# VGLoic/kzg-poly-commit-exploration

Hardware: AMD Instinct MI355X
Metric: g1_msm_commitments_per_sec_degree_2^20 (higher is better)
Workload: dtype i32 digits (Fp: 13 signed radix-2^30 digits, Montgomery 2^390; Fr: 8 x u32, Montgomery 2^256)

## Files before the change

__graft_entry__.py:

```python
import os
import subprocess
import sys

ROOT = os.path.dirname(os.path.abspath(__file__))
sys.path.insert(0, ROOT)
sys.path.insert(0, os.path.join(ROOT, "oracle"))


def build():
    csrc = os.path.join(ROOT, "kzg_poly_commit_exploration_amd", "csrc")
    jobs = str(min(8, os.cpu_count() or 1))
    subprocess.run(["make", "-s", "-C", csrc, "-j", jobs], check=True)
    subprocess.run(["make", "-s", "-C", os.path.join(ROOT, "tests", "device")], check=True)
    subprocess.run(["make", "-s", "-C", os.path.join(ROOT, "tests", "device_columns")], check=True)
    subprocess.run(["make", "-s", "-C", os.path.join(ROOT, "oracle")], check=True)
    for example in ("commit_open", "open_points", "open_combined", "open_sets", "perm_quotient"):
        subprocess.run(["g++", "-std=c++17", "-I" + os.path.join(ROOT, "include"),
                        os.path.join(ROOT, "examples", example + ".cpp"),
                        "-L" + os.path.join(ROOT, "kzg_poly_commit_exploration_amd"), "-lkzg_mi355x",
                        "-Wl,-rpath,$ORIGIN/../kzg_poly_commit_exploration_amd",
                        "-o", os.path.join(ROOT, "examples", example)], check=True)
    import kzg_poly_commit_exploration_amd as K

    K.load_library()


def smoke():
    import numpy as np

    import bigint_twin as T
    import kzg_poly_commit_exploration_amd as K
    import oracle_ctypes as O

    d = 300
    eng = K.SetupArtifactsGenerator(T.BENCH_SECRET_BE).take(d + 1)
    try:
        c = O.bench_coefficients(d + 1)
        z = O.bench_input_point(d)
        y = O.poly_evaluate(c, z)
        srs = O.srs_g1(d + 1, T.BENCH_SECRET_BE)
        rc, want_c = O.commit_naive(c, srs)
        assert rc == 0
        rc, want_p = O.generate_proof(c, z, y, srs)
        assert rc == 0
        poly = K.Polynomial.from_limbs(c)
        got_c = poly.commit(eng)
        got_p = K.Evaluation(K.Scalar.from_limbs(z), K.Scalar.from_limbs(y)).generate_proof(poly, eng)
        assert got_c.compress() == O.p1_compress(want_c), "commitment differs from the oracle"
        assert got_p.compress() == O.p1_compress(want_p), "proof differs from the oracle"
        print("smoke ok: degree %d commit %s proof %s" % (d, got_c.compress().hex()[:16], got_p.compress().hex()[:16]))
    finally:
        eng.close()


if __name__ == "__main__":
    build()
    if len(sys.argv) > 1 and sys.argv[1] == "smoke":
        smoke()
```

kzg_poly_commit_exploration_amd/csrc/msm_sort.hip:

```cpp
#include <cstdlib>
#include <cstring>
#include <type_traits>

#include "engine.h"
#include "fr30.hip.h"
#include "msm_recode.h"

namespace kzg {

typedef uint32_t u32;
#ifndef KZG_DEV
#define KZG_DEV __device__ __forceinline__
#endif

static uint32_t ilog2(uint32_t v) {
    uint32_t b = 0;
    while ((1u << b) < v) b++;
    return b;
}

MsmConfig choose_msm_config(size_t n, size_t table_budget_bytes) {
    const char* force_mode = std::getenv("KZG_MSM_RECODE");
    const char* force_c = std::getenv("KZG_MSM_C");
    const uint32_t fc = force_c ? (uint32_t)std::strtoul(force_c, nullptr, 10) : 0u;
    const bool naf = force_mode && !std::strcmp(force_mode, "naf") && n * 255ull < 0x80000000ull &&
                     (double)n * 255.0 * (double)kAffineBytes <= (double)table_budget_bytes;
    uint32_t best_c = 8;
    const uint32_t best_mode = naf ? kRecodeNaf : kRecodeWindows;
    double best = 1e300;
    for (uint32_t c = 8; c <= (naf ? 21u : 20u); c++) {
        if (fc >= 8 && fc <= (naf ? 21u : 20u) && c != fc) continue;
        if (!naf && !fc && 254u - c * ((255 + c - 1) / c - 1) < 4u) continue;
        double cost = naf ? (double)n * (255.0 / (c + 1) + 0.5) + 8.0 * (double)(1u << (c - 2))
                          : (double)n * ((255 + c - 1) / c) + 20.0 * (double)(1u << (c - 1));
        if (cost < best) {
            best = cost;
            best_c = c;
        }
    }
    MsmConfig cfg;
    cfg.recode = best_mode;
    cfg.c = best_c;
    if (best_mode == kRecodeNaf) {
        cfg.W = 255;
        cfg.level_bits = 1;
        cfg.nb = 1u << (best_c - 2);
        cfg.max_digits = (255 + best_c - 1) / best_c + 1;
    } else {
        cfg.W = (255 + best_c - 1) / best_c;
        cfg.level_bits = best_c;
        cfg.nb = 1u << (best_c - 1);
        cfg.max_digits = cfg.W;
    }
    return cfg;
}

// ... 77 lines not shown
    uint32_t fine_bits = sort_fine_bits(cfg, false);
    uint32_t b = (uint32_t)kMaxCoarse / (cfg.nb >> fine_bits);
    return b < 1 ? 1 : b;
}

uint32_t sort_count_entries(uint32_t max_batch, MsmConfig cfg) {
    uint32_t bins = 0;
    for (uint32_t b = 1; b <= max_batch; b++) {
        const uint32_t nbt = cfg.nb * b;
        const uint32_t q = nbt >> sort_fine_bits(cfg, sort_packed_buckets(nbt, cfg));
        if (q > bins) bins = q;
    }
    return bins * (kMaxTiles + 1u);
}

struct BatchGeom {
    uint32_t n;
    uint32_t batch;
    uint64_t stride;
    uint32_t nb;
};

template <uint32_t C>
__global__ void __launch_bounds__(kRecodeBlock) k_sort_count(const uint32_t* __restrict__ d_scalars, int is_mont,
                                                           BatchGeom bg, MsmConfig cfg, uint32_t tile,
                                                           uint32_t fine_bits, uint32_t coarse_bins,
                                                           uint32_t* __restrict__ d_recoded ,
                                                           uint32_t* __restrict__ d_cnt, uint32_t* __restrict__ d_binfill ,
                                                           uint32_t* __restrict__ d_header) {
    __shared__ u32 s_hist[kMaxCoarse];
    if (blockIdx.x == 0 && threadIdx.x < kHeavyHeaderBytes / 4) d_header[threadIdx.x] = 0;
    for (uint32_t q = threadIdx.x; q < coarse_bins; q += kRecodeBlock) s_hist[q] = 0;
    __syncthreads();
    const uint64_t base = (uint64_t)blockIdx.x * tile;
    const uint64_t total = (uint64_t)bg.n * bg.batch;
    for (uint32_t off = threadIdx.x; off < tile; off += kRecodeBlock) {
        uint64_t g = base + off;
        if (g >= total) break;
        uint32_t p = (uint32_t)(g / bg.n);
        uint32_t i = (uint32_t)(g - (uint64_t)p * bg.n);
        u32 k[8];
        const bool flip = load_scalar(d_scalars, p * bg.stride + i, is_mont, k);
        store_recoded(d_recoded, g, k, flip);
        const u32 pb = p * bg.nb;
        for_each_digit<C>(k, cfg, [&](uint32_t, u32 bkt, bool) { atomicAdd(&s_hist[(pb + bkt) >> fine_bits], 1u); });
    }
    __syncthreads();
    for (uint32_t q = threadIdx.x; q < coarse_bins; q += kRecodeBlock) {
        const u32 c = s_hist[q];
        d_cnt[(size_t)blockIdx.x * coarse_bins + q] = c ? atomicAdd(&d_binfill[q], c) : 0u;
    }
}

template <int N>
__device__ __forceinline__ u32 block_exclusive_scan_n(u32 v, u32* lds, u32& total);
__device__ __forceinline__ u32 block_exclusive_scan_256(u32 v, u32* lds, u32& total);

constexpr uint32_t kFineMaxChunks = 4096;
constexpr uint32_t kFineLocal = 16;
constexpr uint32_t kWsBinStart = 0;
constexpr uint32_t kWsPrefix = kMaxCoarse + 8;
constexpr uint32_t kWsBinFill = 2 * kMaxCoarse + 32;
constexpr uint32_t kWsTable = 3 * kMaxCoarse + 64;
uint32_t sort_workspace_words() { return kWsTable + kFineMaxChunks * (uint32_t)kFineMax + 64; }
uint32_t sort_workspace_zero_words() { return kWsTable; }

template <int BLOCK>
KZG_DEV void spread_tile_cursors(uint32_t coarse_bins, const uint32_t* __restrict__ d_cnt, const uint32_t* __restrict__ d_binfill,
                                 uint32_t ch, uint32_t* __restrict__ d_binstart, uint32_t* __restrict__ d_prefix,
                                 uint32_t* __restrict__ d_total, u32* s_cur , u32* s_scan ) {
    const uint32_t t = threadIdx.x;
    constexpr uint32_t kStripes = kMaxCoarse / BLOCK;
    u32 below[kStripes], all[kStripes];
#pragma unroll
    for (uint32_t s = 0; s < kStripes; s++) {
        const uint32_t q = t + s * BLOCK;
        all[s] = q < coarse_bins ? d_binfill[q] : 0u;
        below[s] = q < coarse_bins ? d_cnt[(size_t)blockIdx.x * coarse_bins + q] : 0u;
    }
    u32 carry = 0, chunk_carry = 0;
#pragma unroll
    for (uint32_t s = 0; s < kStripes; s++) {
        if (s * BLOCK >= coarse_bins) break;
        const uint32_t q = t + s * BLOCK;
        u32 stripe_total;
        const u32 start = carry + block_exclusive_scan_n<BLOCK>(all[s], s_scan, stripe_total);
        __syncthreads();
        if (q < coarse_bins) s_cur[q] = start + below[s];
        if (blockIdx.x == 0) {
            const u32 nch = q < coarse_bins ? (all[s] + ch - 1) / ch : 0u;
            u32 chunk_total;
            const u32 cstart = chunk_carry + block_exclusive_scan_n<BLOCK>(nch, s_scan, chunk_total);
            __syncthreads();
            if (q < coarse_bins) {
                d_binstart[q] = start;
                d_prefix[q] = cstart;
            }
            chunk_carry += chunk_total;
        }
        carry += stripe_total;
    }
    if (blockIdx.x == 0 && t == 0) {
        d_binstart[coarse_bins] = carry;
        d_prefix[coarse_bins] = chunk_carry;
        *d_total = carry;
    }
    __syncthreads();
}

template <uint32_t C>
__global__ void __launch_bounds__(kRecodeBlock) k_sort_spread(const uint32_t* __restrict__ d_recoded,
                                                            BatchGeom bg, uint32_t table_stride, MsmConfig cfg,
                                                            uint32_t tile, uint32_t tiles, uint32_t fine_bits,
                                                            uint32_t coarse_bins, const uint32_t* __restrict__ d_cnt ,
                                                            const uint32_t* __restrict__ d_binfill ,
                                                            uint32_t ch, uint32_t* __restrict__ d_binstart,
                                                            uint32_t* __restrict__ d_prefix, uint32_t* __restrict__ d_total,
                                                            uint64_t* __restrict__ d_pairs, int packed) {
    __shared__ u32 s_cur[kMaxCoarse];
    __shared__ u32 s_scan[kRecodeBlock];
    spread_tile_cursors<kRecodeBlock>(coarse_bins, d_cnt, d_binfill, ch, d_binstart, d_prefix, d_total, s_cur, s_scan);
    const uint64_t base = (uint64_t)blockIdx.x * tile;
    const uint64_t total = (uint64_t)bg.n * bg.batch;
    const u32 fine_mask = (1u << fine_bits) - 1u;
    for (uint32_t off = threadIdx.x; off < tile; off += kRecodeBlock) {
        uint64_t g = base + off;
        if (g >= total) break;
        uint32_t p = (uint32_t)(g / bg.n);
        uint32_t i = (uint32_t)(g - (uint64_t)p * bg.n);
        u32 k[8];
        const bool flip = load_recoded(d_recoded, g, k);
        const u32 pb = p * bg.nb;
        for_each_digit<C>(k, cfg, [&](uint32_t j, u32 bkt, bool neg) {
            u32 b = pb + bkt;
            u32 pos = atomicAdd(&s_cur[b >> fine_bits], 1u);
            u32 ref = (j * table_stride + i) | ((neg != flip) ? 0x80000000u : 0u);
            if (packed) reinterpret_cast<u32*>(d_pairs)[pos] = ref | ((b & fine_mask) << kPackedIndexBits);
            else d_pairs[pos] = ((uint64_t)(b & fine_mask) << 32) | ref;
        });
    }
}

constexpr int kStageBlock = 512;
constexpr uint32_t kStageSlots = 7680;

template <int BLOCK>
KZG_DEV u32 block_exclusive_scan_fast(u32 v, u32* s_wave , u32& total) {
    const uint32_t t = threadIdx.x, lane = t & 63u, w = t >> 6;
    u32 incl = v;
#pragma unroll
    for (uint32_t off = 1; off < 64; off <<= 1) {
        const u32 up = __shfl_up(incl, off, 64);
        if (lane >= off) incl += up;
    }
    if (lane == 63) s_wave[w] = incl;
    __syncthreads();
    u32 base = 0, all = 0;
#pragma unroll
    for (uint32_t i = 0; i < BLOCK / 64; i++) {
        const u32 x = s_wave[i];
        if (i < w) base += x;
        all += x;
    }
    __syncthreads();
    total = all;
    return base + incl - v;
}

template <uint32_t C>
__global__ void __launch_bounds__(kStageBlock) k_sort_spread_staged(const uint32_t* __restrict__ d_recoded,
                                                                  BatchGeom bg, uint32_t table_stride, MsmConfig cfg,
                                                                  uint32_t tile, uint32_t fine_bits, uint32_t coarse_bins,
                                                                  const uint32_t* __restrict__ d_cnt, const uint32_t* __restrict__ d_binfill,
                                                                  uint32_t ch, uint32_t* __restrict__ d_binstart,
                                                                  uint32_t* __restrict__ d_prefix, uint32_t* __restrict__ d_total,
                                                                  uint32_t* __restrict__ d_pairs32) {
    __shared__ u32 s_cur[kMaxCoarse];
    __shared__ u32 s_cnt[kMaxCoarse];
    __shared__ u32 s_gd[kMaxCoarse];
    __shared__ u32 s_scan[kStageBlock];
    __shared__ u32 s_stage[kStageSlots];
    __shared__ uint16_t s_sbin[kStageSlots];
    spread_tile_cursors<kStageBlock>(coarse_bins, d_cnt, d_binfill, ch, d_binstart, d_prefix, d_total, s_cur, s_scan);
    const uint32_t t = threadIdx.x;
    const uint64_t base = (uint64_t)blockIdx.x * tile;
    const uint64_t total = (uint64_t)bg.n * bg.batch;
    const u32 fine_mask = (1u << fine_bits) - 1u;
    const uint32_t per_round = kStageSlots / cfg.max_digits < (uint32_t)kStageBlock ? kStageSlots / cfg.max_digits : (uint32_t)kStageBlock;
    constexpr uint32_t kBinsPerLane = kMaxCoarse / kStageBlock;
    for (uint32_t r0 = 0; r0 < tile; r0 += per_round) {
        for (uint32_t q = t; q < coarse_bins; q += kStageBlock) s_cnt[q] = 0;
        __syncthreads();
        const uint32_t off = r0 + t;
        const uint64_t g = base + off;
        const bool valid = t < per_round && off < tile && g < total;
        u32 k[8];
        bool flip = false;
        uint32_t i = 0;
        u32 pb = 0;
        if (valid) {
            const uint32_t p = (uint32_t)(g / bg.n);
            i = (uint32_t)(g - (uint64_t)p * bg.n);
            pb = p * bg.nb;
            flip = load_recoded(d_recoded, g, k);
            for_each_digit<C>(k, cfg, [&](uint32_t, u32 bkt, bool) { atomicAdd(&s_cnt[(pb + bkt) >> fine_bits], 1u); });
        }
        __syncthreads();
        u32 mine[kBinsPerLane], sum = 0;
#pragma unroll
        for (uint32_t e = 0; e < kBinsPerLane; e++) {
            const uint32_t q = t * kBinsPerLane + e;
            mine[e] = q < coarse_bins ? s_cnt[q] : 0u;
            sum += mine[e];
        }
        u32 round_total;
        u32 run = block_exclusive_scan_fast<kStageBlock>(sum, s_scan, round_total);
#pragma unroll
        for (uint32_t e = 0; e < kBinsPerLane; e++) {
            const uint32_t q = t * kBinsPerLane + e;
            if (q < coarse_bins) {
                const u32 cur = s_cur[q];
                s_gd[q] = cur - run;
                s_cur[q] = cur + mine[e];
                s_cnt[q] = run;
            }
            run += mine[e];
        }
        __syncthreads();
        if (valid) {
            for_each_digit<C>(k, cfg, [&](uint32_t j, u32 bkt, bool neg) {
                const u32 b = pb + bkt, bin = b >> fine_bits;
                const u32 slot = atomicAdd(&s_cnt[bin], 1u);
                s_stage[slot] = (j * table_stride + i) | ((neg != flip) ? 0x80000000u : 0u) | ((b & fine_mask) << kPackedIndexBits);
                s_sbin[slot] = (uint16_t)bin;
            });
        }
        __syncthreads();
        for (uint32_t e = t; e < round_total; e += kStageBlock) d_pairs32[s_gd[s_sbin[e]] + e] = s_stage[e];
    }
}


static uint32_t fine_chunk_len(uint64_t max_pairs) {
    static const uint64_t target = [] {
        const char* v = std::getenv("KZG_FINE_CHUNKS");
        uint64_t t = v ? std::strtoull(v, nullptr, 10) : 2048ull;
        return t < 1 ? 1ull : (t > 2048 ? 2048ull : t);
    }();
    uint64_t ch = (max_pairs + target - 1) / target;
    ch = (ch + 255) / 256 * 256;
    return (uint32_t)(ch < 4096 ? 4096 : ch);
}

struct FineChunk {
    uint32_t bin, beg, end, nch, j, base;
};
KZG_DEV bool locate_chunk(uint32_t k, const uint32_t* __restrict__ d_prefix, const uint32_t* __restrict__ d_binstart,
                          uint32_t coarse_bins, uint32_t ch, FineChunk& c) {
    if (k >= d_prefix[coarse_bins]) return false;
    uint32_t lo = 0, hi = coarse_bins;
    while (hi - lo > 1) {
        uint32_t mid = (lo + hi) >> 1;
        if (d_prefix[mid] <= k) lo = mid; else hi = mid;
    }
    c.bin = lo;
    c.base = d_prefix[lo];
    c.nch = d_prefix[lo + 1] - c.base;
    c.j = k - c.base;
    const uint32_t rs = d_binstart[lo], re = d_binstart[lo + 1];
    c.beg = rs + c.j * ch;
    c.end = (re - c.beg < ch) ? re : c.beg + ch;
    return true;
}

template <bool kPacked> struct SortPair;
template <> struct SortPair<false> {
    typedef uint64_t type;
    static KZG_DEV u32 key(uint64_t p) { return (u32)(p >> 32); }
    static KZG_DEV u32 ref(uint64_t p) { return (u32)p; }
};
template <> struct SortPair<true> {
    typedef uint32_t type;
    static KZG_DEV u32 key(uint32_t p) { return (p >> kPackedIndexBits) & ((1u << kPackedFineBits) - 1u); }
    static KZG_DEV u32 ref(uint32_t p) { return p & (0x80000000u | ((1u << kPackedIndexBits) - 1u)); }
};

template <bool kPacked>
__global__ void __launch_bounds__(kSortBlock) k_fine_count(const typename SortPair<kPacked>::type* __restrict__ d_pairs,
                                                           const uint32_t* __restrict__ d_binstart, uint32_t fine_bits,
                                                           uint32_t coarse_bins, uint32_t ch,
                                                           const uint32_t* __restrict__ d_prefix,
                                                           uint32_t* __restrict__ d_table, uint32_t* __restrict__ d_binfill) {
    __shared__ u32 s_hist[kFineMax];
    if (blockIdx.x == 0)
        for (uint32_t q = threadIdx.x; q < coarse_bins; q += kSortBlock) d_binfill[q] = 0;
    FineChunk c;
    if (!locate_chunk(blockIdx.x, d_prefix, d_binstart, coarse_bins, ch, c)) return;
    const uint32_t fine = 1u << fine_bits;
    if (threadIdx.x < fine) s_hist[threadIdx.x] = 0;
    __syncthreads();
    for (uint32_t e = c.beg + threadIdx.x; e < c.end; e += kSortBlock) atomicAdd(&s_hist[SortPair<kPacked>::key(d_pairs[e])], 1u);
    __syncthreads();
    if (threadIdx.x < fine) d_table[(size_t)c.base * fine + (size_t)threadIdx.x * c.nch + c.j] = s_hist[threadIdx.x];
}

__global__ void __launch_bounds__(kSortBlock) k_fine_binscan(const uint32_t* __restrict__ d_binstart, uint32_t fine_bits,
                                                             const uint32_t* __restrict__ d_prefix,
                                                             uint32_t* __restrict__ d_table, uint32_t* __restrict__ d_offs) {
    __shared__ u32 s_scan[kSortBlock];
    const uint32_t bin = blockIdx.x, t = threadIdx.x;
    const uint32_t fine = 1u << fine_bits;
    const uint32_t base = d_prefix[bin], nch = d_prefix[bin + 1] - base;
    const uint32_t rs = d_binstart[bin];
    if (nch == 0) {
        if (t < fine) d_offs[bin * fine + t] = rs;
        return;
    }
    if (nch <= kFineLocal) return;
    u32* h = d_table + (size_t)base * fine;
    const uint32_t len = fine * nch;
    const uint32_t per = (len + kSortBlock - 1) / kSortBlock;
    const uint32_t lo = t * per < len ? t * per : len, hi = lo + per < len ? lo + per : len;
    u32 sum = 0;
    for (uint32_t i = lo; i < hi; i++) sum += h[i];
    u32 total;
    u32 run = rs + block_exclusive_scan_256(sum, s_scan, total);
    for (uint32_t i = lo; i < hi; i++) {
        const u32 v = h[i];
        h[i] = run;
        run += v;
    }
}

constexpr uint32_t kFineStage = 4096;
template <bool kPacked>
__global__ void __launch_bounds__(kSortBlock) k_fine_scatter(const typename SortPair<kPacked>::type* __restrict__ d_pairs,
                                                             const uint32_t* __restrict__ d_binstart,
                                                             uint32_t fine_bits, uint32_t coarse_bins, uint32_t ch,
                                                             const uint32_t* __restrict__ d_prefix,
                                                             const uint32_t* __restrict__ d_table,
                                                             uint32_t* __restrict__ d_offs,
                                                             uint32_t* __restrict__ d_sorted) {
    __shared__ u32 s_cur[kFineMax];
    __shared__ u32 s_cnt[kFineMax];
    __shared__ u32 s_ref[kFineStage];
    __shared__ u32 s_dst[kFineStage];
    FineChunk c;
    if (!locate_chunk(blockIdx.x, d_prefix, d_binstart, coarse_bins, ch, c)) return;
    const uint32_t fine = 1u << fine_bits;
    const uint32_t t = threadIdx.x;
    {
        u32 mine = 0;
        if (c.nch <= kFineLocal) {
            u32 row = 0, front = 0;
            if (t < fine) {
                const u32* h = d_table + (size_t)c.base * fine + (size_t)t * c.nch;
                for (uint32_t i = 0; i < c.nch; i++) {
                    const u32 v = h[i];
                    row += v;
                    if (i < c.j) front += v;
                }
            }
            u32 total;
            const u32 key_start = d_binstart[c.bin] + block_exclusive_scan_256(row, s_ref, total);
            __syncthreads();
            mine = key_start + front;
            if (c.j == 0 && t < fine) d_offs[c.bin * fine + t] = key_start;
        } else if (t < fine) {
            mine = d_table[(size_t)c.base * fine + (size_t)t * c.nch + c.j];
            if (c.j == 0) d_offs[c.bin * fine + t] = mine;
        }
        if (t < fine) s_cur[t] = mine;
    }
    for (uint32_t r0 = c.beg; r0 < c.end; r0 += kFineStage) {
        const uint32_t r1 = (c.end - r0 < kFineStage) ? c.end : r0 + kFineStage;
        if (t < kFineMax) s_cnt[t] = 0;
        __syncthreads();
        typename SortPair<kPacked>::type pr[kFineStage / kSortBlock];
#pragma unroll
        for (uint32_t q = 0; q < kFineStage / kSortBlock; q++) {
            const uint32_t e = r0 + q * kSortBlock + t;
            pr[q] = e < r1 ? d_pairs[e] : (typename SortPair<kPacked>::type)0;
            if (e < r1) atomicAdd(&s_cnt[SortPair<kPacked>::key(pr[q])], 1u);
        }
        __syncthreads();
        u32 mine = t < kFineMax ? s_cnt[t] : 0u;
        u32 incl = mine;
        __syncthreads();
        if (t < kFineMax) s_ref[t] = incl;
        __syncthreads();
        for (uint32_t off = 1; off < kFineMax; off <<= 1) {
            u32 add = (t < kFineMax && t >= off) ? s_ref[t - off] : 0u;
            __syncthreads();
            if (t < kFineMax) {
                incl += add;
                s_ref[t] = incl;
            }
            __syncthreads();
        }
        const u32 excl = incl - mine;
        u32 gbase = 0;
        if (t < kFineMax) {
            gbase = s_cur[t];
            s_cur[t] = gbase + mine;
            s_cnt[t] = excl;
        }
        __syncthreads();
        if (t < kFineMax) s_dst[t] = gbase - excl;
        __syncthreads();
        u32 keep_dst[kFineStage / kSortBlock];
        u32 keep_pos[kFineStage / kSortBlock];
#pragma unroll
        for (uint32_t q = 0; q < kFineStage / kSortBlock; q++) {
            const uint32_t e = r0 + q * kSortBlock + t;
            if (e < r1) {
                const u32 key = SortPair<kPacked>::key(pr[q]);
                const u32 pos = atomicAdd(&s_cnt[key], 1u);
                keep_pos[q] = pos;
                keep_dst[q] = s_dst[key] + pos;
            }
        }
        __syncthreads();
#pragma unroll
        for (uint32_t q = 0; q < kFineStage / kSortBlock; q++) {
            const uint32_t e = r0 + q * kSortBlock + t;
            if (e < r1) {
                s_ref[keep_pos[q]] = SortPair<kPacked>::ref(pr[q]);
                s_dst[keep_pos[q]] = keep_dst[q];
            }
        }
        __syncthreads();
        const uint32_t cnt = r1 - r0;
        for (uint32_t i = t; i < cnt; i += kSortBlock) d_sorted[s_dst[i]] = s_ref[i];
        __syncthreads();
    }
}

template <int N>
__device__ __forceinline__ u32 block_exclusive_scan_n(u32 v, u32* lds, u32& total) {
    int t = threadIdx.x;
    lds[t] = v;
    __syncthreads();
    for (int off = 1; off < N; off <<= 1) {
        u32 add = t >= off ? lds[t - off] : 0u;
        __syncthreads();
        lds[t] += add;
        __syncthreads();
    }
    total = lds[N - 1];
    return lds[t] - v;
}
__device__ __forceinline__ u32 block_exclusive_scan_256(u32 v, u32* lds, u32& total) { return block_exclusive_scan_n<256>(v, lds, total); }

constexpr uint32_t kSmallSortScalars = 4096;
constexpr uint32_t kSmallSortBuckets = 4096;
constexpr int kSmallSortBlock = 1024;

__global__ void __launch_bounds__(kSmallSortBlock) k_sort_small(const uint32_t* __restrict__ d_scalars, int is_mont, uint32_t n,
                                                                uint32_t table_stride, MsmConfig cfg,
                                                                uint32_t* __restrict__ d_offs,
                                                                uint32_t* __restrict__ d_sorted,
                                                                uint32_t* __restrict__ d_header) {
    __shared__ u32 s_hist[kSmallSortBuckets];
    if (blockIdx.x == 0 && threadIdx.x < kHeavyHeaderBytes / 4) d_header[threadIdx.x] = 0;
    __shared__ u32 s_part[kSmallSortBlock];
    const uint32_t t = threadIdx.x;
    const uint32_t nb = cfg.nb;
    for (uint32_t b = t; b < nb; b += kSmallSortBlock) s_hist[b] = 0;
    __syncthreads();
    for (uint32_t i = t; i < n; i += kSmallSortBlock) {
        u32 k[8];
        (void)load_scalar(d_scalars, i, is_mont, k);
        for_each_digit<0>(k, cfg, [&](uint32_t, u32 bkt, bool) { atomicAdd(&s_hist[bkt], 1u); });
    }
    __syncthreads();
    const uint32_t per = (nb + kSmallSortBlock - 1) / kSmallSortBlock;
    u32 local = 0;
    for (uint32_t q = 0; q < per; q++) {
        uint32_t b = t * per + q;
        if (b < nb) local += s_hist[b];
    }
    s_part[t] = local;
    __syncthreads();
    for (int off = 1; off < kSmallSortBlock; off <<= 1) {
        u32 add = t >= (uint32_t)off ? s_part[t - off] : 0u;
        __syncthreads();
        s_part[t] += add;
        __syncthreads();
    }
    u32 run = s_part[t] - local;
    for (uint32_t q = 0; q < per; q++) {
        uint32_t b = t * per + q;
        if (b < nb) {
            u32 c = s_hist[b];
            d_offs[b] = run;
            s_hist[b] = run;
            run += c;
        }
    }
    if (t == kSmallSortBlock - 1) d_offs[nb] = s_part[t];
    __syncthreads();
    const uint32_t b_lo = (uint32_t)((uint64_t)nb * blockIdx.x / gridDim.x), b_hi = (uint32_t)((uint64_t)nb * (blockIdx.x + 1) / gridDim.x);
    for (uint32_t i = t; i < n; i += kSmallSortBlock) {
        u32 k[8];
        const bool flip = load_scalar(d_scalars, i, is_mont, k);
// ... 72 lines not shown
```

kzg_poly_commit_exploration_amd/csrc/poly_kernels.hip:

```cpp
#include "engine.h"
#include "fr30_host.hpp"

#include <cstring>

namespace kzg {

constexpr int kPolyL = 8;
constexpr int kPolyBlock = 256;
constexpr int kPolyTile = kPolyL * kPolyBlock;

constexpr int kPolyRec = 12;
size_t poly_chunk_words(uint32_t n) { return ((size_t)(n + kPolyTile - 1) / kPolyTile) * kPolyBlock * kPolyRec; }
size_t poly_block_words(uint32_t n) { return ((size_t)(n + kPolyTile - 1) / kPolyTile + 1) * kPolyRec; }

#define KZG_DEV __device__ __forceinline__

struct FrArg {
    int32_t d[kR9];
};
KZG_DEV Fr30 fr_from_arg(const FrArg& a) {
    Fr30 r;
#pragma unroll
    for (int i = 0; i < kR9; i++) r.d[i] = a.d[i];
    return r;
// ... 124 lines not shown
    for (int i = 0; i < kR9; i++) lds[i * kPolyBlock + t] = (uint32_t)H.d[i];
    __syncthreads();
    Fr30 s = fr30_zero();
    if (t + 1 < (uint32_t)kPolyBlock) {
#pragma unroll
        for (int i = 0; i < kR9; i++) s.d[i] = (int32_t)lds[i * kPolyBlock + t + 1];
    }
    for (uint32_t u = hi; u-- > lo;) {
        const Fr30 a = load_rec(d_block + (size_t)u * kPolyRec);
        store_rec(d_block + (size_t)u * kPolyRec, s);
        s = fr30_mul_add(s, zb, a);
    }
    if (t == 0) store_canonical(d_result, fr30_mul(s, fr_from_arg(pw.one)));
}

__global__ void __launch_bounds__(kPolyBlock) k_poly_chunks(const uint32_t* __restrict__ coeffs, uint32_t n, PolyPowers pw,
                                                            uint32_t* __restrict__ d_chunk,
                                                            uint32_t* __restrict__ d_block,
                                                            uint32_t* __restrict__ d_flags) {
    extern __shared__ uint4 lds_tile[];
    __shared__ uint32_t lds[kPolyScanWords];
    const Fr30 z = fr_from_arg(pw.z);
    const uint32_t wave = threadIdx.x >> 6, lane = threadIdx.x & 63;
    uint4* lds_wave = lds_tile + wave * kPolyWaveLds;
    const uint32_t t = blockIdx.x * kPolyBlock + threadIdx.x;
    const uint64_t wave_first = ((uint64_t)blockIdx.x * kPolyBlock + wave * 64u) * kPolyL;
    poly_stage_in(coeffs, wave_first, n, lds_wave, lane);
    Fr30 h = fr30_zero();
    bool nz = false;
#pragma unroll
    for (int k = kPolyL - 1; k >= 0; k--) {
        bool c_nz;
        const Fr30 c = poly_lds_coeff(lds_wave, lane, k, &c_nz);
        if (((uint64_t)t * kPolyL + k) >= 1 && c_nz) nz = true;
        h = fr30_mul_add(h, z, c);
    }
    if (__any(nz) && lane == 0) d_flags[0] = 1u;
    if (t == 0) {
        reinterpret_cast<uint4*>(d_flags + 16)[0] = lds_wave[0];
        reinterpret_cast<uint4*>(d_flags + 16)[1] = lds_wave[1];
    }
    h = block_suffix_scan<kPolyBlock>(h, pw.zl_sq, lds);
    store_planes(d_chunk, (size_t)gridDim.x * kPolyBlock, t, h);
    if (threadIdx.x == 0) store_rec(d_block + (size_t)blockIdx.x * kPolyRec, h);
}

__global__ void __launch_bounds__(kPolyBlock) k_poly_blocks(uint32_t* __restrict__ d_block, uint32_t nblocks, PolyPowers pw,
                                                            uint32_t* __restrict__ d_result) {
    __shared__ uint32_t lds[kPolyScanWords];
    poly_block_stage(d_block, nblocks, pw, d_result, lds);
}

constexpr uint32_t kPolyDirectBlocks = 1024;
KZG_DEV Fr30 poly_carry_from_aggregates(const uint32_t* __restrict__ d_block, uint32_t nblocks, uint32_t first ,
                                        const PolyPowers& pw, uint32_t* lds ) {
    const uint32_t t = threadIdx.x;
    Fr30 sum = fr30_zero();
    if (first + t < nblocks) {
        Fr30 power = fr30_mul(fr_from_arg(pw.ba[t >> 4]), fr_from_arg(pw.bb[t & 15]));
        const Fr30 stride = fr_from_arg(pw.zb256);
        for (uint32_t u = first + t; u < nblocks; u += kPolyBlock) {
            sum = fr30_mul_add(load_rec(d_block + (size_t)u * kPolyRec), power, sum);
            if (u + kPolyBlock < nblocks) power = fr30_mul(power, stride);
        }
    }
    for (int off = kPolyBlock / 2; off >= 1; off >>= 1) {
#pragma unroll
        for (int i = 0; i < kR9; i++) lds[i * kPolyBlock + t] = (uint32_t)sum.d[i];
        __syncthreads();
        if ((int)t < off) {
            Fr30 o;
#pragma unroll
            for (int i = 0; i < kR9; i++) o.d[i] = (int32_t)lds[i * kPolyBlock + t + off];
            sum = fr30_add(sum, o);
        }
        __syncthreads();
    }
#pragma unroll
    for (int i = 0; i < kR9; i++) lds[i * kPolyBlock + t] = (uint32_t)sum.d[i];
    __syncthreads();
    Fr30 total;
#pragma unroll
    for (int i = 0; i < kR9; i++) total.d[i] = (int32_t)lds[i * kPolyBlock];
    return total;
}

__global__ void __launch_bounds__(kPolyBlock) k_poly_apply(const uint32_t* __restrict__ coeffs, uint32_t n, PolyPowers pw,
                                                           const uint32_t* __restrict__ d_chunk,
                                                           const uint32_t* __restrict__ d_block, uint32_t nblocks, int direct,
                                                           uint32_t* __restrict__ d_q, uint32_t* __restrict__ d_result) {
    extern __shared__ uint4 lds_tile[];
    __shared__ uint32_t lds[kPolyScanWords];
    const Fr30 z = fr_from_arg(pw.z);
    const int tl = threadIdx.x;
    const uint32_t wave = threadIdx.x >> 6, lane = threadIdx.x & 63;
    uint4* lds_wave = lds_tile + wave * kPolyWaveLds;
    const uint32_t t = blockIdx.x * kPolyBlock + tl;
    const uint64_t wave_first = ((uint64_t)blockIdx.x * kPolyBlock + wave * 64u) * kPolyL;
    if (d_q) poly_stage_in(coeffs, wave_first, n, lds_wave, lane);
    Fr30 blk_carry;
    if (direct) {
        blk_carry = poly_carry_from_aggregates(d_block, nblocks, blockIdx.x + 1, pw, lds);
        if (blockIdx.x == 0 && tl == 0) {
            const Fr30 s0 = fr30_mul_add(blk_carry, fr_from_arg(pw.zb), load_rec(d_block));
            store_canonical(d_result, fr30_mul(s0, fr_from_arg(pw.one)));
        }
    } else {
        blk_carry = load_rec(d_block + (size_t)blockIdx.x * kPolyRec);
    }
    if (!d_q) return;
    Fr30 h;
    uint32_t dist = (uint32_t)(kPolyBlock - 1 - tl);
    const Fr30 pa = fr_from_arg(pw.pa[dist >> 4]), pb = fr_from_arg(pw.pb[dist & 15]);
    const Fr30 scaled = fr30_mul(blk_carry, fr30_mul(pa, pb));
    if (tl + 1 < kPolyBlock) {
        h = fr30_add(load_planes(d_chunk, (size_t)gridDim.x * kPolyBlock, (size_t)t + 1), scaled);
    } else {
        h = scaled;
    }
#pragma unroll
    for (int k = kPolyL - 1; k >= 0; k--) {
        h = fr30_mul_add(h, z, poly_lds_coeff(lds_wave, lane, k));
        uint32_t l[8];
        fr30_to_limbs(h, l);
        lds_wave[17u * lane + 2u * (uint32_t)k] = make_uint4(l[0], l[1], l[2], l[3]);
        lds_wave[17u * lane + 2u * (uint32_t)k + 1u] = make_uint4(l[4], l[5], l[6], l[7]);
    }
    poly_wave_sync();
    uint4* dst = reinterpret_cast<uint4*>(d_q) + 2 * wave_first;
    const uint64_t valid = wave_first < n ? 2 * ((uint64_t)n - wave_first) : 0;
#pragma unroll
    for (int i = 0; i < 16; i++) {
        const uint32_t g = (uint32_t)i * 64u + lane;
        if (g < valid && (wave_first != 0 || g >= 2)) dst[(int64_t)g - 2] = lds_wave[poly_lds_slot(g)];
    }
}

constexpr uint32_t kPolySingleL = 16;
constexpr uint32_t kPolySingleMax = kPolySingleL * kPolyBlock;
__global__ void __launch_bounds__(kPolyBlock) k_poly_single(const uint32_t* __restrict__ coeffs, uint32_t n, PolyPowers pw,
                                                            uint32_t* __restrict__ d_q, uint32_t* __restrict__ d_small) {
    __shared__ uint32_t lds[kPolyScanWords];
    const Fr30 z = fr_from_arg(pw.z);
    const uint32_t t = threadIdx.x;
    const uint32_t base = t * kPolySingleL;
    Fr30 h = fr30_zero();
    bool nz = false;
#pragma unroll 1
    for (int k = (int)kPolySingleL - 1; k >= 0; k--) {
        const uint32_t idx = base + k;
        Fr30 c = fr30_zero();
        if (idx < n) {
            const uint4* q = reinterpret_cast<const uint4*>(coeffs + (size_t)idx * 8);
            const uint4 lo = q[0], hi = q[1];
            if (idx >= 1 && ((lo.x | lo.y | lo.z | lo.w) | (hi.x | hi.y | hi.z | hi.w)) != 0u) nz = true;
// ... 142 lines not shown
    lds_wave[17u * lane + 2u * (uint32_t)C] = make_uint4(l[0], l[1], l[2], l[3]);
    lds_wave[17u * lane + 2u * (uint32_t)C + 1u] = make_uint4(l[4], l[5], l[6], l[7]);
    if constexpr (C > 0) points_store_sums<C - 1>(acc, one, lds_wave, lane);
}

__global__ void __launch_bounds__(kPolyBlock) k_points_chunks(const uint32_t* __restrict__ coeffs, uint32_t n,
                                                              const PointsRoot* __restrict__ roots, uint32_t k,
                                                              uint32_t* __restrict__ d_block) {
    extern __shared__ uint4 lds_tile[];
    __shared__ uint32_t lds[kPolyScanWords];
    const uint32_t wave = threadIdx.x >> 6, lane = threadIdx.x & 63;
    uint4* lds_wave = lds_tile + wave * kPolyWaveLds;
    const uint64_t wave_first = ((uint64_t)blockIdx.x * kPolyBlock + wave * 64u) * kPolyL;
    poly_stage_in(coeffs, wave_first, n, lds_wave, lane);
    for (uint32_t r = 0; r < k; r++) {
        const Fr30 z = fr_from_arg(roots[r].pw.z);
        Fr30 h = fr30_zero();
#pragma unroll
        for (int c = kPolyL - 1; c >= 0; c--) h = fr30_mul_add(h, z, poly_lds_coeff(lds_wave, lane, c));
        h = block_suffix_scan<kPolyBlock>(h, roots[r].pw.zl_sq, lds);
        if (threadIdx.x == 0) store_rec(d_block + ((size_t)r * gridDim.x + blockIdx.x) * kPolyRec, h);
    }
}

__global__ void __launch_bounds__(kPolyBlock) k_points_blocks(uint32_t* __restrict__ d_block, uint32_t nblocks,
                                                              const PointsRoot* __restrict__ roots,
                                                              uint32_t* __restrict__ d_vals) {
    __shared__ uint32_t lds[kPolyScanWords];
    const uint32_t r = blockIdx.x;
    poly_block_stage(d_block + (size_t)r * nblocks * kPolyRec, nblocks, roots[r].pw, d_vals + 8 * r, lds);
}

__global__ void __launch_bounds__(kPolyBlock) k_points_apply(const uint32_t* __restrict__ coeffs, uint32_t n,
                                                             const PointsRoot* __restrict__ roots, uint32_t k,
                                                             const uint32_t* __restrict__ d_block, uint32_t nblocks, int direct,
                                                             uint32_t* __restrict__ d_q, uint32_t nq,
                                                             uint32_t* __restrict__ d_vals) {
    extern __shared__ uint4 lds_tile[];
    __shared__ uint32_t lds[kPolyScanWords];
    const int tl = threadIdx.x;
    const uint32_t wave = threadIdx.x >> 6, lane = threadIdx.x & 63;
    uint4* lds_wave = lds_tile + wave * kPolyWaveLds;
    const uint64_t wave_first = ((uint64_t)blockIdx.x * kPolyBlock + wave * 64u) * kPolyL;
    if (d_q) poly_stage_in(coeffs, wave_first, n, lds_wave, lane);
    const uint32_t dist = (uint32_t)(kPolyBlock - 1 - tl);
    Fr30 acc[kPolyL];
#pragma unroll
    for (int c = 0; c < kPolyL; c++) acc[c] = fr30_zero();
    for (uint32_t r = 0; r < k; r++) {
        const PolyPowers& pw = roots[r].pw;
        const uint32_t* blk = d_block + (size_t)r * nblocks * kPolyRec;
        Fr30 blk_carry;
        if (direct) {
            blk_carry = poly_carry_from_aggregates(blk, nblocks, blockIdx.x + 1, pw, lds);
            if (blockIdx.x == 0 && tl == 0) {
                const Fr30 s0 = fr30_mul_add(blk_carry, fr_from_arg(pw.zb), load_rec(blk));
                store_canonical(d_vals + 8 * r, fr30_mul(s0, fr_from_arg(pw.one)));
            }
        } else {
            blk_carry = load_rec(blk + (size_t)blockIdx.x * kPolyRec);
        }
        if (!d_q) continue;
        const Fr30 z = fr_from_arg(pw.z);
        Fr30 h = fr30_zero();
#pragma unroll
        for (int c = kPolyL - 1; c >= 0; c--) h = fr30_mul_add(h, z, poly_lds_coeff(lds_wave, lane, c));
        h = block_suffix_scan<kPolyBlock>(h, pw.zl_sq, lds);
#pragma unroll
        for (int i = 0; i < kR9; i++) lds[i * kPolyBlock + tl] = (uint32_t)h.d[i];
        __syncthreads();
        Fr30 next = fr30_zero();
        if (tl + 1 < kPolyBlock) {
#pragma unroll
            for (int i = 0; i < kR9; i++) next.d[i] = (int32_t)lds[i * kPolyBlock + tl + 1];
        }
        __syncthreads();
        const Fr30 pa = fr_from_arg(pw.pa[dist >> 4]), pb = fr_from_arg(pw.pb[dist & 15]);
        h = fr30_add(next, fr30_mul(blk_carry, fr30_mul(pa, pb)));
        points_replay<kPolyL - 1>(acc, h, z, fr_from_arg(roots[r].w), lds_wave, lane);
    }
    if (!d_q) return;
    points_store_sums<kPolyL - 1>(acc, fr_from_arg(roots[0].pw.one), lds_wave, lane);
    poly_wave_sync();
    uint4* dst = reinterpret_cast<uint4*>(d_q) + 2 * wave_first;
    const uint64_t end = 2 * ((uint64_t)nq + 1);
    const uint64_t valid = wave_first < nq + 1 ? end - 2 * wave_first : 0;
#pragma unroll
    for (int i = 0; i < 16; i++) {
        const uint32_t g = (uint32_t)i * 64u + lane;
        if (g < valid && (wave_first != 0 || g >= 2)) dst[(int64_t)g - 2] = lds_wave[poly_lds_slot(g)];
    }
}

bool points_prepare_device() {
    const bool a = hipFuncSetAttribute((const void*)k_points_chunks, hipFuncAttributeMaxDynamicSharedMemorySize, (int)kPolyTileLds) == hipSuccess;
    const bool b = hipFuncSetAttribute((const void*)k_points_apply, hipFuncAttributeMaxDynamicSharedMemorySize, (int)kPolyTileLds) == hipSuccess;
    if (!(a && b)) (void)hipGetLastError();
    return a && b;
}

void points_fill_roots(void* h_roots, const uint64_t* zs_mont, const uint64_t* ws_mont, uint32_t k, uint32_t n) {
    PointsRoot* roots = static_cast<PointsRoot*>(h_roots);
    for (uint32_t r = 0; r < k; r++) {
        std::memset(&roots[r], 0, sizeof roots[r]);
        uint32_t zw[8];
        std::memcpy(zw, zs_mont + 4 * r, 32);
        poly_powers(roots[r].pw, zw, n);
// ... 23 lines not shown
    h = fr30_mul_add(h, z, poly_lds_coeff(lds_wave, lane, C));
    acc[C] = fr30_add(acc[C], h);
    __builtin_amdgcn_sched_barrier(0);
    if constexpr (C > 0) sets_replay<C - 1>(acc, h, z, lds_wave, lane);
}

__global__ void __launch_bounds__(kPolyBlock) k_sets_chunks(const uint32_t* __restrict__ d_g, uint32_t n,
                                                            const PointsRoot* __restrict__ roots, uint32_t k,
                                                            uint32_t* __restrict__ d_block) {
    extern __shared__ uint4 lds_tile[];
    __shared__ uint32_t lds[kPolyScanWords];
    const uint32_t wave = threadIdx.x >> 6, lane = threadIdx.x & 63;
    uint4* lds_wave = lds_tile + wave * kPolyWaveLds;
    const uint64_t wave_first = ((uint64_t)blockIdx.x * kPolyBlock + wave * 64u) * kPolyL;
    for (uint32_t r = 0; r < k; r++) {
        poly_wave_sync();
        poly_stage_in(d_g + 8 * (size_t)r * n, wave_first, n, lds_wave, lane);
        const Fr30 z = fr_from_arg(roots[r].pw.z);
        Fr30 h = fr30_zero();
#pragma unroll
        for (int c = kPolyL - 1; c >= 0; c--) h = fr30_mul_add(h, z, poly_lds_coeff(lds_wave, lane, c));
        h = block_suffix_scan<kPolyBlock>(h, roots[r].pw.zl_sq, lds);
        if (threadIdx.x == 0) store_rec(d_block + ((size_t)r * gridDim.x + blockIdx.x) * kPolyRec, h);
    }
}

__global__ void __launch_bounds__(kPolyBlock) k_sets_blocks(uint32_t* __restrict__ d_block, uint32_t nblocks,
                                                            const PointsRoot* __restrict__ roots,
                                                            uint32_t* __restrict__ d_vals) {
    __shared__ uint32_t lds[kPolyScanWords];
    const uint32_t r = blockIdx.x;
    poly_block_stage(d_block + (size_t)r * nblocks * kPolyRec, nblocks, roots[r].pw, d_vals + 8 * r, lds);
}

__global__ void __launch_bounds__(kPolyBlock) k_sets_apply(const uint32_t* __restrict__ d_g, uint32_t n,
                                                           const PointsRoot* __restrict__ roots, uint32_t k,
                                                           const uint32_t* __restrict__ d_block, uint32_t nblocks, int direct,
                                                           uint32_t* __restrict__ d_q, uint32_t nq) {
    extern __shared__ uint4 lds_tile[];
    __shared__ uint32_t lds[kPolyScanWords];
    const int tl = threadIdx.x;
    const uint32_t wave = threadIdx.x >> 6, lane = threadIdx.x & 63;
    uint4* lds_wave = lds_tile + wave * kPolyWaveLds;
    const uint64_t wave_first = ((uint64_t)blockIdx.x * kPolyBlock + wave * 64u) * kPolyL;
    const uint32_t dist = (uint32_t)(kPolyBlock - 1 - tl);
    Fr30 acc[kPolyL];
#pragma unroll
    for (int c = 0; c < kPolyL; c++) acc[c] = fr30_zero();
    for (uint32_t r = 0; r < k; r++) {
        const PolyPowers& pw = roots[r].pw;
        const uint32_t* blk = d_block + (size_t)r * nblocks * kPolyRec;
        poly_wave_sync();
        poly_stage_in(d_g + 8 * (size_t)r * n, wave_first, n, lds_wave, lane);
        const Fr30 blk_carry = direct ? poly_carry_from_aggregates(blk, nblocks, blockIdx.x + 1, pw, lds)
                                      : load_rec(blk + (size_t)blockIdx.x * kPolyRec);
        const Fr30 z = fr_from_arg(pw.z);
        Fr30 h = fr30_zero();
#pragma unroll
        for (int c = kPolyL - 1; c >= 0; c--) h = fr30_mul_add(h, z, poly_lds_coeff(lds_wave, lane, c));
        h = block_suffix_scan<kPolyBlock>(h, pw.zl_sq, lds);
#pragma unroll
        for (int i = 0; i < kR9; i++) lds[i * kPolyBlock + tl] = (uint32_t)h.d[i];
        __syncthreads();
        Fr30 next = fr30_zero();
        if (tl + 1 < kPolyBlock) {
#pragma unroll
            for (int i = 0; i < kR9; i++) next.d[i] = (int32_t)lds[i * kPolyBlock + tl + 1];
        }
        __syncthreads();
        const Fr30 pa = fr_from_arg(pw.pa[dist >> 4]), pb = fr_from_arg(pw.pb[dist & 15]);
        h = fr30_add(next, fr30_mul(blk_carry, fr30_mul(pa, pb)));
        sets_replay<kPolyL - 1>(acc, h, z, lds_wave, lane);
    }
    points_store_sums<kPolyL - 1>(acc, fr_from_arg(roots[0].pw.one), lds_wave, lane);
    poly_wave_sync();
    uint4* dst = reinterpret_cast<uint4*>(d_q) + 2 * wave_first;
    const uint64_t end = 2 * ((uint64_t)nq + 1);
    const uint64_t valid = wave_first < (uint64_t)nq + 1 ? end - 2 * wave_first : 0;
#pragma unroll
    for (int i = 0; i < 16; i++) {
        const uint32_t g = (uint32_t)i * 64u + lane;
        if (g < valid && (wave_first != 0 || g >= 2)) dst[(int64_t)g - 2] = lds_wave[poly_lds_slot(g)];
    }
}

bool sets_prepare_device() {
    const bool a = hipFuncSetAttribute((const void*)k_sets_chunks, hipFuncAttributeMaxDynamicSharedMemorySize, (int)kPolyTileLds) == hipSuccess;
    const bool b = hipFuncSetAttribute((const void*)k_sets_apply, hipFuncAttributeMaxDynamicSharedMemorySize, (int)kPolyTileLds) == hipSuccess;
    if (!(a && b)) (void)hipGetLastError();
    return a && b;
}

void launch_quotient_sets(hipStream_t s, const uint32_t* d_g, uint32_t n, const void* d_roots, uint32_t k, uint32_t* d_q,
                          uint32_t* d_block, uint32_t* d_vals) {
    if (n < 2 || k == 0) return;
    const PointsRoot* roots = static_cast<const PointsRoot*>(d_roots);
    const uint32_t nblocks = (n + kPolyTile - 1) / kPolyTile;
    hipLaunchKernelGGL(k_sets_chunks, dim3(nblocks), dim3(kPolyBlock), kPolyTileLds, s, d_g, n, roots, k, d_block);
    const int direct = nblocks <= kPolyDirectBlocks;
    if (!direct) hipLaunchKernelGGL(k_sets_blocks, dim3(k), dim3(kPolyBlock), 0, s, d_block, nblocks, roots, d_vals);
    hipLaunchKernelGGL(k_sets_apply, dim3(nblocks), dim3(kPolyBlock), kPolyTileLds, s, d_g, n, roots, k, d_block, nblocks, direct,
                       d_q, n - 1);
}

}
```

Before: 438.0.

## Replace LDS Hillis-Steele block scans with wave-shuffle scans and fewer barriers

Replaces the LDS-based log-step block scans in the MSM sort kernels (spread cursors, fine binscan, fine scatter) with a wave-shuffle scan plus per-wave totals. The two scans in block 0 of the spread kernel are fused into one pass, and each stripe gets its own scratch so the trailing barrier can be dropped. The Fr30 tree reduction in the polynomial carry path becomes a shuffle reduction followed by a small cross-wave sum. The aim is to cut __syncthreads and LDS traffic in the sort and scan phases; skipping barriers relies on the scratch never being reused while other threads still read it.

```diff
diff --git a/__graft_entry__.py b/__graft_entry__.py
--- a/__graft_entry__.py
+++ b/__graft_entry__.py
@@ -13,6 +13,7 @@
     subprocess.run(["make", "-s", "-C", csrc, "-j", jobs], check=True)
     subprocess.run(["make", "-s", "-C", os.path.join(ROOT, "tests", "device")], check=True)
     subprocess.run(["make", "-s", "-C", os.path.join(ROOT, "tests", "device_columns")], check=True)
+    subprocess.run(["make", "-s", "-C", os.path.join(ROOT, "tests", "device_scan")], check=True)
     subprocess.run(["make", "-s", "-C", os.path.join(ROOT, "oracle")], check=True)
     for example in ("commit_open", "open_points", "open_combined", "open_sets", "perm_quotient"):
         subprocess.run(["g++", "-std=c++17", "-I" + os.path.join(ROOT, "include"),
diff --git a/kzg_poly_commit_exploration_amd/csrc/block_scan.hip.h b/kzg_poly_commit_exploration_amd/csrc/block_scan.hip.h
--- /dev/null
+++ b/kzg_poly_commit_exploration_amd/csrc/block_scan.hip.h
@@ -0,0 +1,51 @@
+#pragma once
+#include <hip/hip_runtime.h>
+#include <stdint.h>
+
+namespace kzg {
+
+template <int BLOCK, int K, bool kFenceAfter>
+__device__ __forceinline__ void block_exclusive_scans_fast(uint32_t (&v)[K], uint32_t* s_wave, uint32_t (&total)[K]) {
+    static_assert(BLOCK % 64 == 0 && BLOCK >= 64 && K >= 1, "whole waves");
+    constexpr uint32_t kWaves = BLOCK / 64;
+    const uint32_t t = threadIdx.x, lane = t & 63u, w = t >> 6;
+    uint32_t incl[K];
+#pragma unroll
+    for (int k = 0; k < K; k++) incl[k] = v[k];
+#pragma unroll
+    for (uint32_t off = 1; off < 64; off <<= 1) {
+#pragma unroll
+        for (int k = 0; k < K; k++) {
+            const uint32_t up = __shfl_up(incl[k], off, 64);
+            if (lane >= off) incl[k] += up;
+        }
+    }
+    if (lane == 63) {
+#pragma unroll
+        for (int k = 0; k < K; k++) s_wave[k * kWaves + w] = incl[k];
+    }
+    __syncthreads();
+#pragma unroll
+    for (int k = 0; k < K; k++) {
+        uint32_t base = 0, all = 0;
+#pragma unroll
+        for (uint32_t i = 0; i < kWaves; i++) {
+            const uint32_t x = s_wave[k * kWaves + i];
+            if (i < w) base += x;
+            all += x;
+        }
+        total[k] = all;
+        v[k] = base + incl[k] - v[k];
+    }
+    if (kFenceAfter) __syncthreads();
+}
+
+template <int BLOCK, bool kFenceAfter>
+__device__ __forceinline__ uint32_t block_exclusive_scan_fast(uint32_t v, uint32_t* s_wave , uint32_t& total) {
+    uint32_t a[1] = {v}, tot[1];
+    block_exclusive_scans_fast<BLOCK, 1, kFenceAfter>(a, s_wave, tot);
+    total = tot[0];
+    return a[0];
+}
+
+}
diff --git a/kzg_poly_commit_exploration_amd/csrc/msm_sort.hip b/kzg_poly_commit_exploration_amd/csrc/msm_sort.hip
--- a/kzg_poly_commit_exploration_amd/csrc/msm_sort.hip
+++ b/kzg_poly_commit_exploration_amd/csrc/msm_sort.hip
@@ -2,6 +2,7 @@
 #include <cstring>
 #include <type_traits>
 
+#include "block_scan.hip.h"
 #include "engine.h"
 #include "fr30.hip.h"
 #include "msm_recode.h"
@@ -185,10 +186,6 @@
     }
 }
 
-template <int N>
-__device__ __forceinline__ u32 block_exclusive_scan_n(u32 v, u32* lds, u32& total);
-__device__ __forceinline__ u32 block_exclusive_scan_256(u32 v, u32* lds, u32& total);
-
 constexpr uint32_t kFineMaxChunks = 4096;
 constexpr uint32_t kFineLocal = 16;
 constexpr uint32_t kWsBinStart = 0;
@@ -199,11 +196,14 @@
 uint32_t sort_workspace_zero_words() { return kWsTable; }
 
 template <int BLOCK>
+constexpr uint32_t spread_scan_words() { return (kMaxCoarse / BLOCK) * 2 * (BLOCK / 64); }
+template <int BLOCK>
 KZG_DEV void spread_tile_cursors(uint32_t coarse_bins, const uint32_t* __restrict__ d_cnt, const uint32_t* __restrict__ d_binfill,
                                  uint32_t ch, uint32_t* __restrict__ d_binstart, uint32_t* __restrict__ d_prefix,
                                  uint32_t* __restrict__ d_total, u32* s_cur , u32* s_scan ) {
     const uint32_t t = threadIdx.x;
     constexpr uint32_t kStripes = kMaxCoarse / BLOCK;
+    constexpr uint32_t kStripeWords = 2 * (BLOCK / 64);
     u32 below[kStripes], all[kStripes];
 #pragma unroll
     for (uint32_t s = 0; s < kStripes; s++) {
@@ -216,22 +216,23 @@
     for (uint32_t s = 0; s < kStripes; s++) {
         if (s * BLOCK >= coarse_bins) break;
         const uint32_t q = t + s * BLOCK;
-        u32 stripe_total;
-        const u32 start = carry + block_exclusive_scan_n<BLOCK>(all[s], s_scan, stripe_total);
-        __syncthreads();
-        if (q < coarse_bins) s_cur[q] = start + below[s];
         if (blockIdx.x == 0) {
-            const u32 nch = q < coarse_bins ? (all[s] + ch - 1) / ch : 0u;
-            u32 chunk_total;
-            const u32 cstart = chunk_carry + block_exclusive_scan_n<BLOCK>(nch, s_scan, chunk_total);
-            __syncthreads();
+            u32 v[2] = {all[s], q < coarse_bins ? (all[s] + ch - 1) / ch : 0u}, sum[2];
+            block_exclusive_scans_fast<BLOCK, 2, false>(v, s_scan + s * kStripeWords, sum);
+            const u32 start = carry + v[0];
             if (q < coarse_bins) {
+                s_cur[q] = start + below[s];
                 d_binstart[q] = start;
-                d_prefix[q] = cstart;
+                d_prefix[q] = chunk_carry + v[1];
             }
-            chunk_carry += chunk_total;
-        }
-        carry += stripe_total;
+            carry += sum[0];
+            chunk_carry += sum[1];
+        } else {
+            u32 stripe_total;
+            const u32 start = carry + block_exclusive_scan_fast<BLOCK, false>(all[s], s_scan + s * kStripeWords, stripe_total);
+            if (q < coarse_bins) s_cur[q] = start + below[s];
+            carry += stripe_total;
+        }
     }
     if (blockIdx.x == 0 && t == 0) {
         d_binstart[coarse_bins] = carry;
@@ -251,7 +252,7 @@
                                                             uint32_t* __restrict__ d_prefix, uint32_t* __restrict__ d_total,
                                                             uint64_t* __restrict__ d_pairs, int packed) {
     __shared__ u32 s_cur[kMaxCoarse];
-    __shared__ u32 s_scan[kRecodeBlock];
+    __shared__ u32 s_scan[spread_scan_words<kRecodeBlock>()];
     spread_tile_cursors<kRecodeBlock>(coarse_bins, d_cnt, d_binfill, ch, d_binstart, d_prefix, d_total, s_cur, s_scan);
     const uint64_t base = (uint64_t)blockIdx.x * tile;
     const uint64_t total = (uint64_t)bg.n * bg.batch;
@@ -277,29 +278,6 @@
 constexpr int kStageBlock = 512;
 constexpr uint32_t kStageSlots = 7680;
 
-template <int BLOCK>
-KZG_DEV u32 block_exclusive_scan_fast(u32 v, u32* s_wave , u32& total) {
-    const uint32_t t = threadIdx.x, lane = t & 63u, w = t >> 6;
-    u32 incl = v;
-#pragma unroll
-    for (uint32_t off = 1; off < 64; off <<= 1) {
-        const u32 up = __shfl_up(incl, off, 64);
-        if (lane >= off) incl += up;
-    }
-    if (lane == 63) s_wave[w] = incl;
-    __syncthreads();
-    u32 base = 0, all = 0;
-#pragma unroll
-    for (uint32_t i = 0; i < BLOCK / 64; i++) {
-        const u32 x = s_wave[i];
-        if (i < w) base += x;
-        all += x;
-    }
-    __syncthreads();
-    total = all;
-    return base + incl - v;
-}
-
 template <uint32_t C>
 __global__ void __launch_bounds__(kStageBlock) k_sort_spread_staged(const uint32_t* __restrict__ d_recoded,
                                                                   BatchGeom bg, uint32_t table_stride, MsmConfig cfg,
@@ -311,7 +289,7 @@
     __shared__ u32 s_cur[kMaxCoarse];
     __shared__ u32 s_cnt[kMaxCoarse];
     __shared__ u32 s_gd[kMaxCoarse];
-    __shared__ u32 s_scan[kStageBlock];
+    __shared__ u32 s_scan[spread_scan_words<kStageBlock>()];
     __shared__ u32 s_stage[kStageSlots];
     __shared__ uint16_t s_sbin[kStageSlots];
     spread_tile_cursors<kStageBlock>(coarse_bins, d_cnt, d_binfill, ch, d_binstart, d_prefix, d_total, s_cur, s_scan);
@@ -347,7 +325,7 @@
             sum += mine[e];
         }
         u32 round_total;
-        u32 run = block_exclusive_scan_fast<kStageBlock>(sum, s_scan, round_total);
+        u32 run = block_exclusive_scan_fast<kStageBlock, false>(sum, s_scan, round_total);
 #pragma unroll
         for (uint32_t e = 0; e < kBinsPerLane; e++) {
             const uint32_t q = t * kBinsPerLane + e;
@@ -440,7 +418,7 @@
 __global__ void __launch_bounds__(kSortBlock) k_fine_binscan(const uint32_t* __restrict__ d_binstart, uint32_t fine_bits,
                                                              const uint32_t* __restrict__ d_prefix,
                                                              uint32_t* __restrict__ d_table, uint32_t* __restrict__ d_offs) {
-    __shared__ u32 s_scan[kSortBlock];
+    __shared__ u32 s_scan[kSortBlock / 64];
     const uint32_t bin = blockIdx.x, t = threadIdx.x;
     const uint32_t fine = 1u << fine_bits;
     const uint32_t base = d_prefix[bin], nch = d_prefix[bin + 1] - base;
@@ -457,7 +435,7 @@
     u32 sum = 0;
     for (uint32_t i = lo; i < hi; i++) sum += h[i];
     u32 total;
-    u32 run = rs + block_exclusive_scan_256(sum, s_scan, total);
+    u32 run = rs + block_exclusive_scan_fast<kSortBlock, false>(sum, s_scan, total);
     for (uint32_t i = lo; i < hi; i++) {
         const u32 v = h[i];
         h[i] = run;
@@ -474,10 +452,12 @@
                                                              const uint32_t* __restrict__ d_table,
                                                              uint32_t* __restrict__ d_offs,
                                                              uint32_t* __restrict__ d_sorted) {
+    static_assert(kSortBlock == kFineMax, "one lane per fine key: lane t alone touches s_cur[t] and scans s_cnt[t]");
     __shared__ u32 s_cur[kFineMax];
     __shared__ u32 s_cnt[kFineMax];
     __shared__ u32 s_ref[kFineStage];
     __shared__ u32 s_dst[kFineStage];
+    __shared__ u32 s_scan[kSortBlock / 64];
     FineChunk c;
     if (!locate_chunk(blockIdx.x, d_prefix, d_binstart, coarse_bins, ch, c)) return;
     const uint32_t fine = 1u << fine_bits;
@@ -495,8 +475,7 @@
                 }
             }
             u32 total;
-            const u32 key_start = d_binstart[c.bin] + block_exclusive_scan_256(row, s_ref, total);
-            __syncthreads();
+            const u32 key_start = d_binstart[c.bin] + block_exclusive_scan_fast<kSortBlock, false>(row, s_scan, total);
             mine = key_start + front;
             if (c.j == 0 && t < fine) d_offs[c.bin * fine + t] = key_start;
         } else if (t < fine) {
@@ -507,7 +486,7 @@
     }
     for (uint32_t r0 = c.beg; r0 < c.end; r0 += kFineStage) {
         const uint32_t r1 = (c.end - r0 < kFineStage) ? c.end : r0 + kFineStage;
-        if (t < kFineMax) s_cnt[t] = 0;
+        s_cnt[t] = 0;
         __syncthreads();
         typename SortPair<kPacked>::type pr[kFineStage / kSortBlock];
 #pragma unroll
@@ -517,29 +496,13 @@
             if (e < r1) atomicAdd(&s_cnt[SortPair<kPacked>::key(pr[q])], 1u);
         }
         __syncthreads();
-        u32 mine = t < kFineMax ? s_cnt[t] : 0u;
-        u32 incl = mine;
-        __syncthreads();
-        if (t < kFineMax) s_ref[t] = incl;
-        __syncthreads();
-        for (uint32_t off = 1; off < kFineMax; off <<= 1) {
-            u32 add = (t < kFineMax && t >= off) ? s_ref[t - off] : 0u;
-            __syncthreads();
-            if (t < kFineMax) {
-                incl += add;
-                s_ref[t] = incl;
-            }
-            __syncthreads();
-        }
-        const u32 excl = incl - mine;
-        u32 gbase = 0;
-        if (t < kFineMax) {
-            gbase = s_cur[t];
-            s_cur[t] = gbase + mine;
-            s_cnt[t] = excl;
-        }
-        __syncthreads();
-        if (t < kFineMax) s_dst[t] = gbase - excl;
+        const u32 mine = s_cnt[t];
+        u32 round_total;
+        const u32 excl = block_exclusive_scan_fast<kSortBlock, false>(mine, s_scan, round_total);
+        const u32 gbase = s_cur[t];
+        s_cur[t] = gbase + mine;
+        s_cnt[t] = excl;
+        s_dst[t] = gbase - excl;
         __syncthreads();
         u32 keep_dst[kFineStage / kSortBlock];
         u32 keep_pos[kFineStage / kSortBlock];
@@ -565,25 +528,8 @@
         __syncthreads();
         const uint32_t cnt = r1 - r0;
         for (uint32_t i = t; i < cnt; i += kSortBlock) d_sorted[s_dst[i]] = s_ref[i];
-        __syncthreads();
-    }
-}
-
-template <int N>
-__device__ __forceinline__ u32 block_exclusive_scan_n(u32 v, u32* lds, u32& total) {
-    int t = threadIdx.x;
-    lds[t] = v;
-    __syncthreads();
-    for (int off = 1; off < N; off <<= 1) {
-        u32 add = t >= off ? lds[t - off] : 0u;
-        __syncthreads();
-        lds[t] += add;
-        __syncthreads();
-    }
-    total = lds[N - 1];
-    return lds[t] - v;
-}
-__device__ __forceinline__ u32 block_exclusive_scan_256(u32 v, u32* lds, u32& total) { return block_exclusive_scan_n<256>(v, lds, total); }
+    }
+}
 
 constexpr uint32_t kSmallSortScalars = 4096;
 constexpr uint32_t kSmallSortBuckets = 4096;
diff --git a/kzg_poly_commit_exploration_amd/csrc/poly_kernels.hip b/kzg_poly_commit_exploration_amd/csrc/poly_kernels.hip
--- a/kzg_poly_commit_exploration_amd/csrc/poly_kernels.hip
+++ b/kzg_poly_commit_exploration_amd/csrc/poly_kernels.hip
@@ -200,9 +200,11 @@
 }
 
 constexpr uint32_t kPolyDirectBlocks = 1024;
+template <bool kFenceAfter>
 KZG_DEV Fr30 poly_carry_from_aggregates(const uint32_t* __restrict__ d_block, uint32_t nblocks, uint32_t first ,
                                         const PolyPowers& pw, uint32_t* lds ) {
-    const uint32_t t = threadIdx.x;
+    const uint32_t t = threadIdx.x, lane = t & 63u, wave = t >> 6;
+    constexpr uint32_t kWaves = kPolyBlock / 64;
     Fr30 sum = fr30_zero();
     if (first + t < nblocks) {
         Fr30 power = fr30_mul(fr_from_arg(pw.ba[t >> 4]), fr_from_arg(pw.bb[t & 15]));
@@ -212,24 +214,29 @@
             if (u + kPolyBlock < nblocks) power = fr30_mul(power, stride);
         }
     }
-    for (int off = kPolyBlock / 2; off >= 1; off >>= 1) {
-#pragma unroll
-        for (int i = 0; i < kR9; i++) lds[i * kPolyBlock + t] = (uint32_t)sum.d[i];
-        __syncthreads();
-        if ((int)t < off) {
-            Fr30 o;
-#pragma unroll
-            for (int i = 0; i < kR9; i++) o.d[i] = (int32_t)lds[i * kPolyBlock + t + off];
-            sum = fr30_add(sum, o);
-        }
-        __syncthreads();
-    }
-#pragma unroll
-    for (int i = 0; i < kR9; i++) lds[i * kPolyBlock + t] = (uint32_t)sum.d[i];
+#pragma unroll
+    for (int off = 32; off >= 1; off >>= 1) {
+        Fr30 o;
+#pragma unroll
+        for (int i = 0; i < kR9; i++) o.d[i] = __shfl_down(sum.d[i], off, 64);
+        sum = fr30_add(sum, o);
+    }
+    if (lane == 0) {
+#pragma unroll
+        for (int i = 0; i < kR9; i++) lds[wave * kR9 + i] = (uint32_t)sum.d[i];
+    }
     __syncthreads();
     Fr30 total;
 #pragma unroll
-    for (int i = 0; i < kR9; i++) total.d[i] = (int32_t)lds[i * kPolyBlock];
+    for (int i = 0; i < kR9; i++) total.d[i] = (int32_t)lds[i];
+#pragma unroll
+    for (uint32_t w = 1; w < kWaves; w++) {
+        Fr30 o;
+#pragma unroll
+        for (int i = 0; i < kR9; i++) o.d[i] = (int32_t)lds[w * kR9 + i];
+        total = fr30_add(total, o);
+    }
+    if (kFenceAfter) __syncthreads();
     return total;
 }
 
@@ -248,7 +255,7 @@
     if (d_q) poly_stage_in(coeffs, wave_first, n, lds_wave, lane);
     Fr30 blk_carry;
     if (direct) {
-        blk_carry = poly_carry_from_aggregates(d_block, nblocks, blockIdx.x + 1, pw, lds);
+        blk_carry = poly_carry_from_aggregates<false>(d_block, nblocks, blockIdx.x + 1, pw, lds);
         if (blockIdx.x == 0 && tl == 0) {
             const Fr30 s0 = fr30_mul_add(blk_carry, fr_from_arg(pw.zb), load_rec(d_block));
             store_canonical(d_result, fr30_mul(s0, fr_from_arg(pw.one)));
@@ -497,7 +504,7 @@
         const uint32_t* blk = d_block + (size_t)r * nblocks * kPolyRec;
         Fr30 blk_carry;
         if (direct) {
-            blk_carry = poly_carry_from_aggregates(blk, nblocks, blockIdx.x + 1, pw, lds);
+            blk_carry = poly_carry_from_aggregates<true>(blk, nblocks, blockIdx.x + 1, pw, lds);
             if (blockIdx.x == 0 && tl == 0) {
                 const Fr30 s0 = fr30_mul_add(blk_carry, fr_from_arg(pw.zb), load_rec(blk));
                 store_canonical(d_vals + 8 * r, fr30_mul(s0, fr_from_arg(pw.one)));
@@ -627,7 +634,7 @@
         const uint32_t* blk = d_block + (size_t)r * nblocks * kPolyRec;
         poly_wave_sync();
         poly_stage_in(d_g + 8 * (size_t)r * n, wave_first, n, lds_wave, lane);
-        const Fr30 blk_carry = direct ? poly_carry_from_aggregates(blk, nblocks, blockIdx.x + 1, pw, lds)
+        const Fr30 blk_carry = direct ? poly_carry_from_aggregates<true>(blk, nblocks, blockIdx.x + 1, pw, lds)
                                       : load_rec(blk + (size_t)blockIdx.x * kPolyRec);
         const Fr30 z = fr_from_arg(pw.z);
         Fr30 h = fr30_zero();
```

Result: no change. 435.0 (-0.7%).
